# Cardinal-Cryptography/zk-apps

Measured on AMD Instinct MI355X. Metric: shielder_withdraw_groth16_proofs_per_sec_2^20_constraints, higher is better.
Workload: dtype int: signed 28-bit limbs in 32-bit words, 64-bit column accumulators (Fr 255-bit / Fq 381-bit Montgomery); 1 GPU; single withdraw-shaped Groth16 proof, N=2^20 (7 Fr NTTs, 4 G1 MSM + 1 G2 MSM of 2^20-1 terms), 1 proof per step per GPU; relation=update_note (withdraw) with Poseidon-5 hashing, chain-padded to N, curve=BLS12-381, independent_proofs_per_rank=173, distinct_witnesses_per_rank=64, fresh_r_s_per_proof=True, proofs_in_flight_per_gpu=3, msm_schedule=A | B1 (over r*z) + L + H reduced together | B2 (G2)

## Files before the change

zk-apps_amd/csrc/ntt.hip:

```cpp
#include <stdlib.h>
#include <type_traits>
#include <utility>
#include "ntt.hpp"
#include "tune.hpp"

namespace zkmi {

namespace {

__device__ __forceinline__ void ld_words8(const uint32_t* p, uint32_t* w) {
  const uint4* q = reinterpret_cast<const uint4*>(p);
  const uint4 a = q[0], b = q[1];
  w[0] = a.x; w[1] = a.y; w[2] = a.z; w[3] = a.w;
  w[4] = b.x; w[5] = b.y; w[6] = b.z; w[7] = b.w;
}
__device__ __forceinline__ void st_words8(uint32_t* p, const uint32_t* w) {
  uint4* q = reinterpret_cast<uint4*>(p);
  q[0] = make_uint4(w[0], w[1], w[2], w[3]);
  q[1] = make_uint4(w[4], w[5], w[6], w[7]);
}

template <class F>
__global__ void k_bitrev_copy(const F* __restrict__ in, F* __restrict__ out, int log_n) {
  const uint32_t i = blockIdx.x * blockDim.x + threadIdx.x;
  if (i >= (1u << log_n)) return;
  const uint32_t r = log_n ? (__brev(i) >> (32 - log_n)) : 0u;
  st28(out + r, ld28(in + i));
}

template <class F, bool DIF, bool LOCAL_TW, int THREADS>
__global__ void __launch_bounds__(THREADS)
k_ntt_pass(F* __restrict__ data, const F* __restrict__ tw, int log_n, int t0, int S, int Q,
           const F* __restrict__ post, uint32_t* __restrict__ canon_out) {
  data += (size_t)blockIdx.y << log_n;
  if (canon_out) canon_out += ((size_t)blockIdx.y << log_n) * 8;
  extern __shared__ __align__(16) unsigned char lds_raw[];
  F* tile = reinterpret_cast<F*>(lds_raw);
  const uint32_t tile_n = 1u << (S + Q);
  F* ctw = tile + tile_n;
  const uint32_t blk = blockIdx.x;
  const uint32_t mid_bits = (t0 > 0) ? (uint32_t)(t0 - Q) : 0u;
  const uint32_t mid = blk & ((1u << mid_bits) - 1u);
  const uint32_t hi = blk >> mid_bits;
  const uint32_t qeff = (t0 > 0) ? (uint32_t)Q : 0u;
  auto gindex = [&](uint32_t L) -> uint32_t {
    if (t0 == 0) return blk * tile_n + L;
    const uint32_t e = L >> Q, c = L & ((1u << Q) - 1u);
    return (hi << (t0 + S)) | (e << t0) | (mid << Q) | c;
  };
  auto twist = [&](uint32_t L) -> F {
    const uint32_t e = L >> Q, c = L & ((1u << Q) - 1u);
    const uint32_t col = (mid << Q) | c;
    const uint32_t ex = (col * (__brev(e) >> (32 - S))) << (log_n - t0 - S);
    const uint32_t halfn = 1u << (log_n - 1);
    F f = ld28(tw + (ex & (halfn - 1u)));
    return (ex & halfn) ? f.neg() : f;
  };
  if (LOCAL_TW)
    for (uint32_t k = threadIdx.x; k < (1u << (S - 1)); k += THREADS) ctw[k] = ld28(tw + ((size_t)k << (log_n - S)));
  for (uint32_t L = threadIdx.x; L < tile_n; L += THREADS) {
    F v = ld28(data + gindex(L));
    if (LOCAL_TW && !DIF && t0 > 0) v = v * twist(L);
    tile[L] = v;
  }
  __syncthreads();

  const uint32_t half = tile_n >> 1;
  for (int s = 0; s < S; s++) {
    const int u = DIF ? (S - 1 - s) : s;
    const int t = t0 + u;
    const uint32_t dist_log = (uint32_t)u + qeff;
    const uint32_t dist = 1u << dist_log;
    for (uint32_t b = threadIdx.x; b < half; b += THREADS) {
      const uint32_t lo = b & (dist - 1u);
      const uint32_t L0 = ((b >> dist_log) << (dist_log + 1)) | lo;
      const uint32_t L1 = L0 | dist;
      F w;
      if (LOCAL_TW) {
        w = ctw[(lo >> qeff) << (S - 1 - u)];
      } else {
        const uint32_t j = gindex(L0) & ((1u << t) - 1u);
        w = ld28(tw + ((size_t)j << (log_n - 1 - t)));
      }
      const F x = tile[L0];
      if (DIF) {
        const F y = tile[L1];
        tile[L0] = x + y;
        tile[L1] = x.sub_lazy(y) * w;
      } else {
        const F y = tile[L1] * w;
        tile[L0] = x + y;
        tile[L1] = x - y;
      }
    }
    __syncthreads();
  }

  for (uint32_t L = threadIdx.x; L < tile_n; L += THREADS) {
    const uint32_t g = gindex(L);
    F v = tile[L];
    if (LOCAL_TW && DIF && t0 > 0) v = v * twist(L);
    if (post) v = v * ld28(post + g);
    if (canon_out) {
      uint32_t w[8];
      v.to_canonical(w);
      st_words8(canon_out + (size_t)g * 8, w);
    } else {
      st28(data + g, v);
    }
  }
}

#ifdef ZKMI_EXPERIMENTS
#include "ntt_exp.hpp"
#endif

template <class F>
__global__ void __launch_bounds__(256)
k_mul_table(F* __restrict__ a, const F* __restrict__ b, uint32_t n) {
  const uint32_t i = blockIdx.x * blockDim.x + threadIdx.x;
  if (i < n) st28(a + i, ld28(a + i) * ld28(b + i));
}

template <class F>
__global__ void __launch_bounds__(256)
k_scale(F* __restrict__ a, F s, uint32_t n) {
  const uint32_t i = blockIdx.x * blockDim.x + threadIdx.x;
  if (i < n) st28(a + i, ld28(a + i) * s);
}

template <class F>
__global__ void __launch_bounds__(256)
k_power_table(F* __restrict__ out, F base, F first, uint32_t n) {
  const uint32_t i0 = (blockIdx.x * blockDim.x + threadIdx.x) * 16u;
  if (i0 >= n) return;
  F v = first, sq = base;
  for (uint32_t e = i0; e; e >>= 1) {
    if (e & 1u) v = v * sq;
    sq = sq * sq;
  }
  for (uint32_t k = 0; k < 16u && i0 + k < n; k++) {
    st28(out + i0 + k, v);
    v = v * base;
  }
}

template <class F>
__global__ void __launch_bounds__(256)
k_from_canonical(const uint32_t* __restrict__ in, F* __restrict__ out, uint32_t n) {
  const uint32_t i = blockIdx.x * blockDim.x + threadIdx.x;
  if (i >= n) return;
  uint32_t w[8];
  ld_words8(in + (size_t)i * 8, w);
  st28(out + i, F::from_canonical(w));
}
template <class F>
__global__ void __launch_bounds__(256)
k_to_canonical(const F* __restrict__ in, uint32_t* __restrict__ out, uint32_t n) {
  const uint32_t i = blockIdx.x * blockDim.x + threadIdx.x;
  if (i >= n) return;
  uint32_t w[8];
  ld28(in + i).to_canonical(w);
  st_words8(out + (size_t)i * 8, w);
}

}

Fr fr_root_of_unity(int log_n) {
  static const uint32_t ROOT_2_32[8] = {0x439f0d2bu, 0x3829971fu, 0x8c2280b9u, 0xb6368350u,
                                        0x22c813b4u, 0xd09b6819u, 0xdfe81f20u, 0x16a2a19eu};
  Fr w;
  for (int i = 0; i < 8; i++) w.l[i] = ROOT_2_32[i];
  w = w.to_mont();
  for (int i = 32; i > log_n; i--) w = w.sqr();
  return w;
}

NttField<Fr28>::Host NttField<Fr28>::root_max() { return fr_root_of_unity(32); }
NttField<BnFr28>::Host NttField<BnFr28>::root_max() {
  static const uint32_t ROOT_2_28[8] = {0x60c37c9cu, 0xd34f1ed9u, 0xd39329c8u, 0x3215cf6du,
                                        0x3dd31f74u, 0x98865ea9u, 0x166d18b7u, 0x03ddb9f5u};
  BnFr w;
  for (int i = 0; i < 8; i++) w.l[i] = ROOT_2_28[i];
  return w.to_mont();
}

template <class H>
static H host_from_u64(uint64_t v) {
  H a = H::zero();
  a.l[0] = (uint32_t)v;
  a.l[1] = (uint32_t)(v >> 32);
  return a.to_mont();
}
template <class F, class H>
static F to28(const H& a) {
  H c = a.from_mont();
  return F::from_canonical(c.l);
}

template <class F>
NttDomainT<F>::~NttDomainT() {
  F* ptrs[] = {tw_fwd, tw_inv, coset_fwd, coset_inv_n, rev_coset_n, rev_coset_inv_n, n_inv, scratch};
  for (F* p : ptrs)
    if (p) (void)hipFree(p);
}

template <class F>
hipError_t NttDomainT<F>::init(int log_n_, hipStream_t stream) {
  using H = typename NttField<F>::Host;
  if (log_n_ > NttField<F>::TWO_ADICITY) return hipErrorInvalidValue;
  log_n = log_n_;
  const uint32_t n = 1u << log_n;
  const uint32_t half = n > 1 ? n / 2 : 1;
  hipError_t e;
  F** alloc_n[] = {&coset_fwd, &coset_inv_n, &rev_coset_n, &rev_coset_inv_n, &scratch};
  if ((e = hipMalloc(&tw_fwd, sizeof(F) * half)) != hipSuccess) return e;
  if ((e = hipMalloc(&tw_inv, sizeof(F) * half)) != hipSuccess) return e;
  if ((e = hipMalloc(&n_inv, sizeof(F))) != hipSuccess) return e;
  for (F** p : alloc_n)
    if ((e = hipMalloc(p, sizeof(F) * n)) != hipSuccess) return e;
  H w = NttField<F>::root_max();
  for (int i = NttField<F>::TWO_ADICITY; i > log_n; i--) w = w.sqr();
  const H g = host_from_u64<H>(7);
  const H ninv = host_from_u64<H>(n).inv();
  const F one28 = F::one(), ninv28 = to28<F, H>(ninv);
  n_inv_host = ninv28;
  const int T = 256;
  auto blocks = [&](uint32_t cnt) { return (cnt + 16 * T - 1) / (16 * T); };
  hipLaunchKernelGGL(k_power_table<F>, dim3(blocks(half)), dim3(T), 0, stream, tw_fwd, to28<F, H>(w), one28, half);
  hipLaunchKernelGGL(k_power_table<F>, dim3(blocks(half)), dim3(T), 0, stream, tw_inv, to28<F, H>(w.inv()), one28, half);
  hipLaunchKernelGGL(k_power_table<F>, dim3(blocks(n)), dim3(T), 0, stream, coset_fwd, to28<F, H>(g), one28, n);
  hipLaunchKernelGGL(k_power_table<F>, dim3(blocks(n)), dim3(T), 0, stream, coset_inv_n, to28<F, H>(g.inv()), ninv28, n);
  hipLaunchKernelGGL(k_power_table<F>, dim3(blocks(n)), dim3(T), 0, stream, scratch, to28<F, H>(g), ninv28, n);
  hipLaunchKernelGGL(k_bitrev_copy<F>, dim3((n + T - 1) / T), dim3(T), 0, stream, scratch, rev_coset_n, log_n);
  hipLaunchKernelGGL(k_bitrev_copy<F>, dim3((n + T - 1) / T), dim3(T), 0, stream, coset_inv_n, rev_coset_inv_n, log_n);
  if ((e = hipMemcpyAsync(n_inv, &ninv28, sizeof(F), hipMemcpyHostToDevice, stream)) != hipSuccess) return e;
  if ((e = hipStreamSynchronize(stream)) != hipSuccess) return e;
  return hipGetLastError();
}

static int ntt_rb_mode() { return ZK_TUNE("ZKMI_NTT_RB", 6); }

#ifdef ZKMI_EXPERIMENTS
template <class F, bool DIF, bool LTW, int LOGE, int LOGR = 0, bool ONEW = false>
static void launch_rb(dim3 grid, uint32_t tile_n, int S, hipStream_t stream, F* buf, const F* tw, int log_n, int t0, int Q,
                      const F* post, uint32_t* canon_out) {
  const size_t words = (size_t)F::NL * (tile_n + (tile_n >> 5)) +
                       (LTW ? (size_t)F::NL * ((1u << (S - 1)) + ((1u << (S - 1)) >> 5) + 1u) : 0u);
  hipLaunchKernelGGL((k_ntt_pass_rb<F, DIF, LTW, LOGE, LOGR, ONEW>), grid, dim3(tile_n >> (LOGE + LOGR)), words * sizeof(uint32_t), stream,
                     buf, tw, log_n, t0, S, Q, post, canon_out);
}
#endif

template <class F, bool DIF>
static hipError_t run_passes(F* buf, const F* tw, int log_n, const F* post, uint32_t* canon_out,
                             hipStream_t stream, uint32_t batch = 1) {
  const uint32_t n = 1u << log_n;
  int mode = ntt_rb_mode();
  if (mode == 5 && log_n < 9) mode = 3;
  const int rb = (mode == 1 || mode == 2 || mode == 4 || mode == 5) ? mode : 0;
  const int tile_log = mode == 5 ? 9 : mode == 4 ? 10 : 11;
  struct Pass {
    int t0, S, Q;
  } passes[4];
  int np = 0;
  const int max_s = mode == 5 ? 9 : 10;
  const int want_np = (log_n + max_s - 1) / max_s;
  for (int t0 = 0; t0 < log_n;) {
    int S = log_n - t0;
    if (S > max_s) S = max_s;
    if (mode == 5) {
      const int left = want_np - np;
      S = (log_n - t0 + left - 1) / left;
    }
    int Q;
    if (rb) {
      Q = tile_log - S;
      const int room = (t0 > 0) ? t0 : (log_n - S);
      if (Q > room) Q = room;
    } else {
      Q = (t0 > 0) ? 1 : ((log_n > S) ? 1 : 0);
      if ((mode == 3 || mode == 6) && t0 > 0 && S < 10 && log_n - 11 >= 9) Q = (11 - S < t0) ? 11 - S : t0;
      if (mode == 6 && S + Q == 11) Q -= 1;
    }
    passes[np++] = {t0, S, Q};
    t0 += S;
  }
  const bool local3 = ZK_TUNE("ZKMI_NTT_LOCAL3", 0) == 1;
  const bool local_tw = np <= 2 || mode == 5 || local3;
  for (int k = 0; k < np; k++) {
    const Pass& p = DIF ? passes[np - 1 - k] : passes[k];
    const bool last = (k == np - 1);
    const uint32_t tile_n = 1u << (p.S + p.Q);
    const uint32_t nblk = n / tile_n;
    const F* pp = last ? post : nullptr;
    uint32_t* co = last ? canon_out : nullptr;
    const dim3 grid(nblk, batch);
#ifdef ZKMI_EXPERIMENTS
    if (rb == 5) {
      launch_rb<F, DIF, true, 2, 1, true>(grid, tile_n, p.S, stream, buf, tw, log_n, p.t0, p.Q, pp, co);
      continue;
    }
    if (rb == 4 && tile_n == 1024) {
      if (local_tw) launch_rb<F, DIF, true, 2, 2>(grid, tile_n, p.S, stream, buf, tw, log_n, p.t0, p.Q, pp, co);
      else launch_rb<F, DIF, false, 2, 2>(grid, tile_n, p.S, stream, buf, tw, log_n, p.t0, p.Q, pp, co);
      continue;
    }
    if (rb && rb != 4 && rb != 5 && tile_n >= 512) {
      if (rb == 2) {
        if (local_tw) launch_rb<F, DIF, true, 2>(grid, tile_n, p.S, stream, buf, tw, log_n, p.t0, p.Q, pp, co);
        else launch_rb<F, DIF, false, 2>(grid, tile_n, p.S, stream, buf, tw, log_n, p.t0, p.Q, pp, co);
      } else {
        if (local_tw) launch_rb<F, DIF, true, 3>(grid, tile_n, p.S, stream, buf, tw, log_n, p.t0, p.Q, pp, co);
        else launch_rb<F, DIF, false, 3>(grid, tile_n, p.S, stream, buf, tw, log_n, p.t0, p.Q, pp, co);
      }
      continue;
    }
#endif
    const size_t lds = ((size_t)tile_n + (local_tw ? (1u << (p.S - 1)) : 0u)) * sizeof(F);
    if (tile_n == 1024 && mode == 6) {
      if (local_tw)
        hipLaunchKernelGGL((k_ntt_pass<F, DIF, true, 512>), grid, dim3(512), lds, stream, buf, tw, log_n, p.t0, p.S, p.Q, pp, co);
      else
        hipLaunchKernelGGL((k_ntt_pass<F, DIF, false, 512>), grid, dim3(512), lds, stream, buf, tw, log_n, p.t0, p.S, p.Q, pp, co);
    } else if (tile_n >= 1024) {
      if (local_tw)
        hipLaunchKernelGGL((k_ntt_pass<F, DIF, true, 1024>), grid, dim3(1024), lds, stream, buf, tw, log_n, p.t0, p.S,
                           p.Q, pp, co);
      else
        hipLaunchKernelGGL((k_ntt_pass<F, DIF, false, 1024>), grid, dim3(1024), lds, stream, buf, tw, log_n, p.t0,
                           p.S, p.Q, pp, co);
    } else if (local_tw) {
      hipLaunchKernelGGL((k_ntt_pass<F, DIF, true, 64>), grid, dim3(64), lds, stream, buf, tw, log_n, p.t0, p.S, p.Q,
                         pp, co);
    } else {
      hipLaunchKernelGGL((k_ntt_pass<F, DIF, false, 64>), grid, dim3(64), lds, stream, buf, tw, log_n, p.t0, p.S, p.Q,
                         pp, co);
    }
  }
  return hipGetLastError();
}

template <class F>
hipError_t NttDomainT<F>::inverse_to_rev(F* d, const F* post_table, uint32_t* canon_out, hipStream_t st, uint32_t batch) {
  if (log_n == 0) {
    if (batch != 1) return hipErrorInvalidValue;
    if (post_table) hipLaunchKernelGGL(k_mul_table<F>, dim3(1), dim3(256), 0, st, d, post_table, 1u);
    if (canon_out) hipLaunchKernelGGL(k_to_canonical<F>, dim3(1), dim3(256), 0, st, d, canon_out, 1u);
    return hipGetLastError();
  }
  return run_passes<F, true>(d, tw_inv, log_n, post_table, canon_out, st, batch);
}

template <class F>
hipError_t NttDomainT<F>::forward_from_rev(F* d, hipStream_t st, uint32_t batch) {
  if (log_n == 0) return hipSuccess;
  return run_passes<F, false>(d, tw_fwd, log_n, nullptr, nullptr, st, batch);
}

template <class F>
hipError_t NttDomainT<F>::transform(F* d_data, bool inverse, bool coset, hipStream_t stream) {
  const uint32_t n = 1u << log_n;
  const int T = 256;
  if (coset && !inverse)
    hipLaunchKernelGGL(k_mul_table<F>, dim3((n + T - 1) / T), dim3(T), 0, stream, d_data, coset_fwd, n);
  if (log_n > 0) {
    hipLaunchKernelGGL(k_bitrev_copy<F>, dim3((n + T - 1) / T), dim3(T), 0, stream, d_data, scratch, log_n);
    hipError_t e = run_passes<F, false>(scratch, inverse ? tw_inv : tw_fwd, log_n, nullptr, nullptr, stream);
    if (e != hipSuccess) return e;
    if ((e = hipMemcpyAsync(d_data, scratch, sizeof(F) * n, hipMemcpyDeviceToDevice, stream)) != hipSuccess) return e;
  }
  if (inverse) {
    if (coset) {
      hipLaunchKernelGGL(k_mul_table<F>, dim3((n + T - 1) / T), dim3(T), 0, stream, d_data, coset_inv_n, n);
    } else {
      hipLaunchKernelGGL(k_scale<F>, dim3((n + T - 1) / T), dim3(T), 0, stream, d_data, n_inv_host, n);
    }
  }
  return hipGetLastError();
}

template <class F>
hipError_t ntt_from_canonical(const uint32_t* d_in, F* d_out, uint32_t n, hipStream_t s) {
  if (!n) return hipSuccess;
  hipLaunchKernelGGL(k_from_canonical<F>, dim3((n + 63) / 64), dim3(64), 0, s, d_in, d_out, n);
  return hipGetLastError();
}
template <class F>
hipError_t ntt_to_canonical(const F* d_in, uint32_t* d_out, uint32_t n, hipStream_t s) {
  if (!n) return hipSuccess;
  hipLaunchKernelGGL(k_to_canonical<F>, dim3((n + 255) / 256), dim3(256), 0, s, d_in, d_out, n);
  return hipGetLastError();
}
template <class F>
hipError_t ntt_mul_table(F* d, const F* table, uint32_t n, hipStream_t s) {
  if (!n) return hipSuccess;
  hipLaunchKernelGGL(k_mul_table<F>, dim3((n + 255) / 256), dim3(256), 0, s, d, table, n);
  return hipGetLastError();
}

#ifdef ZKMI_EXPERIMENTS
template <class F>
static hipError_t rb_enable_big_lds() {
  const void* fns[] = {reinterpret_cast<const void*>(k_ntt_pass_rb<F, true, true, 3>),  reinterpret_cast<const void*>(k_ntt_pass_rb<F, false, true, 3>),
                       reinterpret_cast<const void*>(k_ntt_pass_rb<F, true, false, 3>), reinterpret_cast<const void*>(k_ntt_pass_rb<F, false, false, 3>),
                       reinterpret_cast<const void*>(k_ntt_pass_rb<F, true, true, 2>),  reinterpret_cast<const void*>(k_ntt_pass_rb<F, false, true, 2>),
                       reinterpret_cast<const void*>(k_ntt_pass_rb<F, true, false, 2>), reinterpret_cast<const void*>(k_ntt_pass_rb<F, false, false, 2>),
                       reinterpret_cast<const void*>((k_ntt_pass_rb<F, true, true, 2, 2>)),  reinterpret_cast<const void*>((k_ntt_pass_rb<F, false, true, 2, 2>)),
                       reinterpret_cast<const void*>((k_ntt_pass_rb<F, true, false, 2, 2>)), reinterpret_cast<const void*>((k_ntt_pass_rb<F, false, false, 2, 2>)),
                       reinterpret_cast<const void*>((k_ntt_pass_rb<F, true, true, 2, 1, true>)), reinterpret_cast<const void*>((k_ntt_pass_rb<F, false, true, 2, 1, true>))};
  for (const void* f : fns) {
    const hipError_t e = hipFuncSetAttribute(f, hipFuncAttributeMaxDynamicSharedMemorySize, 160 * 1024);
    if (e != hipSuccess) return e;
  }
  return hipSuccess;
}
#endif

hipError_t ntt_enable_big_lds() {
  const void* fns[] = {reinterpret_cast<const void*>(k_ntt_pass<Fr28, true, true, 1024>),
                       reinterpret_cast<const void*>(k_ntt_pass<Fr28, false, true, 1024>),
                       reinterpret_cast<const void*>(k_ntt_pass<Fr28, true, false, 1024>),
                       reinterpret_cast<const void*>(k_ntt_pass<Fr28, false, false, 1024>),
                       reinterpret_cast<const void*>(k_ntt_pass<BnFr28, true, true, 1024>),
                       reinterpret_cast<const void*>(k_ntt_pass<BnFr28, false, true, 1024>),
                       reinterpret_cast<const void*>(k_ntt_pass<BnFr28, true, false, 1024>),
                       reinterpret_cast<const void*>(k_ntt_pass<BnFr28, false, false, 1024>),
                       reinterpret_cast<const void*>(k_ntt_pass<Fr28, true, true, 512>),
                       reinterpret_cast<const void*>(k_ntt_pass<Fr28, false, true, 512>),
                       reinterpret_cast<const void*>(k_ntt_pass<Fr28, true, false, 512>),
                       reinterpret_cast<const void*>(k_ntt_pass<Fr28, false, false, 512>),
                       reinterpret_cast<const void*>(k_ntt_pass<BnFr28, true, true, 512>),
                       reinterpret_cast<const void*>(k_ntt_pass<BnFr28, false, true, 512>),
                       reinterpret_cast<const void*>(k_ntt_pass<BnFr28, true, false, 512>),
                       reinterpret_cast<const void*>(k_ntt_pass<BnFr28, false, false, 512>)};
  for (const void* f : fns) {
    hipError_t e = hipFuncSetAttribute(f, hipFuncAttributeMaxDynamicSharedMemorySize, 160 * 1024);
    if (e != hipSuccess) return e;
  }
#ifdef ZKMI_EXPERIMENTS
  hipError_t e = rb_enable_big_lds<Fr28>();
  if (e == hipSuccess) e = rb_enable_big_lds<BnFr28>();
  return e;
#else
  return hipSuccess;
#endif
}

template struct NttDomainT<Fr28>;
template struct NttDomainT<BnFr28>;
template hipError_t ntt_from_canonical<Fr28>(const uint32_t*, Fr28*, uint32_t, hipStream_t);
template hipError_t ntt_to_canonical<Fr28>(const Fr28*, uint32_t*, uint32_t, hipStream_t);
template hipError_t ntt_mul_table<Fr28>(Fr28*, const Fr28*, uint32_t, hipStream_t);
template hipError_t ntt_from_canonical<BnFr28>(const uint32_t*, BnFr28*, uint32_t, hipStream_t);
template hipError_t ntt_to_canonical<BnFr28>(const BnFr28*, uint32_t*, uint32_t, hipStream_t);
template hipError_t ntt_mul_table<BnFr28>(BnFr28*, const BnFr28*, uint32_t, hipStream_t);

}
```

Baseline: 59.57 proofs/s.

## Use lazy limb reduction in NTT butterflies and fuse unit stages into load/store

NTT butterflies now use lazy add/sub on signed limbs and only carry-normalize every few stages (every 2 for DIF, every 3 for DIT), so most per-stage carry work is skipped. The twiddle-free unit-distance stage is folded into the global load (DIT) or the final store (DIF), which removes one LDS round-trip and one barrier per pass. Sign flips on twiddles become branchless XOR negation. This relies on the limb headroom being large enough for several unnormalized additions, and the multiply must accept unnormalized inputs.

```diff
diff --git a/zk-apps_amd/csrc/ntt.hip b/zk-apps_amd/csrc/ntt.hip
--- a/zk-apps_amd/csrc/ntt.hip
+++ b/zk-apps_amd/csrc/ntt.hip
@@ -26,6 +26,18 @@
   if (i >= (1u << log_n)) return;
   const uint32_t r = log_n ? (__brev(i) >> (32 - log_n)) : 0u;
   st28(out + r, ld28(in + i));
+}
+
+constexpr int NTT_DIF_SWEEP = 2;
+constexpr int NTT_DIT_SWEEP = 3;
+
+template <class F>
+__device__ __forceinline__ F neg_if_lazy(const F& f, bool sign) {
+  const int32_t m = sign ? -1 : 0;
+  F r;
+#pragma unroll
+  for (int i = 0; i < F::NL; i++) r.l[i] = (f.l[i] ^ m) - m;
+  return r;
 }
 
 template <class F, bool DIF, bool LOCAL_TW, int THREADS>
@@ -53,31 +65,49 @@
     const uint32_t col = (mid << Q) | c;
     const uint32_t ex = (col * (__brev(e) >> (32 - S))) << (log_n - t0 - S);
     const uint32_t halfn = 1u << (log_n - 1);
-    F f = ld28(tw + (ex & (halfn - 1u)));
-    return (ex & halfn) ? f.neg() : f;
+    return neg_if_lazy(ld28(tw + (ex & (halfn - 1u))), (ex & halfn) != 0u);
   };
+  const bool twisted = LOCAL_TW && t0 > 0;
+  const bool unit_stage = LOCAL_TW || t0 == 0;
+  const uint32_t half = tile_n >> 1;
+  const uint32_t unit_dist = 1u << qeff;
+  auto lower = [](uint32_t b, uint32_t dl) -> uint32_t { return ((b >> dl) << (dl + 1)) | (b & ((1u << dl) - 1u)); };
+  auto sweeps = [&](int s) -> bool { return (s + 1) % (DIF ? NTT_DIF_SWEEP : NTT_DIT_SWEEP) == 0 || s == S - 1; };
+
   if (LOCAL_TW)
     for (uint32_t k = threadIdx.x; k < (1u << (S - 1)); k += THREADS) ctw[k] = ld28(tw + ((size_t)k << (log_n - S)));
-  for (uint32_t L = threadIdx.x; L < tile_n; L += THREADS) {
-    F v = ld28(data + gindex(L));
-    if (LOCAL_TW && !DIF && t0 > 0) v = v * twist(L);
-    tile[L] = v;
+  if (!DIF && unit_stage) {
+    for (uint32_t b = threadIdx.x; b < half; b += THREADS) {
+      const uint32_t L0 = lower(b, qeff), L1 = L0 | unit_dist;
+      F x = ld28(data + gindex(L0)), y = ld28(data + gindex(L1));
+      if (twisted) {
+        x = x * twist(L0);
+        y = y * twist(L1);
+      }
+      F a = x.add_lazy(y), d = x.sub_lazy(y);
+      if (sweeps(0)) {
+        a.carry();
+        d.carry();
+      }
+      tile[L0] = a;
+      tile[L1] = d;
+    }
+  } else {
+    for (uint32_t L = threadIdx.x; L < tile_n; L += THREADS) tile[L] = ld28(data + gindex(L));
   }
   __syncthreads();
 
-  const uint32_t half = tile_n >> 1;
-  for (int s = 0; s < S; s++) {
+  auto stage = [&](int s, auto SWEEP) {
     const int u = DIF ? (S - 1 - s) : s;
     const int t = t0 + u;
     const uint32_t dist_log = (uint32_t)u + qeff;
     const uint32_t dist = 1u << dist_log;
     for (uint32_t b = threadIdx.x; b < half; b += THREADS) {
-      const uint32_t lo = b & (dist - 1u);
-      const uint32_t L0 = ((b >> dist_log) << (dist_log + 1)) | lo;
+      const uint32_t L0 = lower(b, dist_log);
       const uint32_t L1 = L0 | dist;
       F w;
       if (LOCAL_TW) {
-        w = ctw[(lo >> qeff) << (S - 1 - u)];
+        w = ctw[((L0 & (dist - 1u)) >> qeff) << (S - 1 - u)];
       } else {
         const uint32_t j = gindex(L0) & ((1u << t) - 1u);
         w = ld28(tw + ((size_t)j << (log_n - 1 - t)));
@@ -85,28 +115,65 @@
       const F x = tile[L0];
       if (DIF) {
         const F y = tile[L1];
-        tile[L0] = x + y;
+        F a = x.add_lazy(y);
+        if (decltype(SWEEP)::value) a.carry();
+        tile[L0] = a;
         tile[L1] = x.sub_lazy(y) * w;
       } else {
         const F y = tile[L1] * w;
-        tile[L0] = x + y;
-        tile[L1] = x - y;
+        F a = x.add_lazy(y), d = x.sub_lazy(y);
+        if (decltype(SWEEP)::value) {
+          a.carry();
+          d.carry();
+        }
+        tile[L0] = a;
+        tile[L1] = d;
       }
     }
     __syncthreads();
-  }
-
-  for (uint32_t L = threadIdx.x; L < tile_n; L += THREADS) {
-    const uint32_t g = gindex(L);
-    F v = tile[L];
-    if (LOCAL_TW && DIF && t0 > 0) v = v * twist(L);
-    if (post) v = v * ld28(post + g);
+  };
+  const int s_begin = (!DIF && unit_stage) ? 1 : 0, s_end = (DIF && unit_stage) ? S - 1 : S;
+  for (int s = s_begin; s < s_end; s++) {
+    if (sweeps(s)) stage(s, std::true_type());
+    else stage(s, std::false_type());
+  }
+
+  auto store = [&](uint32_t g, const F& v) {
     if (canon_out) {
       uint32_t w[8];
       v.to_canonical(w);
       st_words8(canon_out + (size_t)g * 8, w);
     } else {
       st28(data + g, v);
+    }
+  };
+  if (DIF && unit_stage) {
+    for (uint32_t b = threadIdx.x; b < half; b += THREADS) {
+      const uint32_t L0 = lower(b, qeff), L1 = L0 | unit_dist;
+      const uint32_t g0 = gindex(L0), g1 = gindex(L1);
+      const F x = tile[L0], y = tile[L1];
+      F a = x.add_lazy(y), d = x.sub_lazy(y);
+      if (twisted) {
+        a = a * twist(L0);
+        d = d * twist(L1);
+      }
+      if (post) {
+        a = a * ld28(post + g0);
+        d = d * ld28(post + g1);
+      }
+      if (!twisted && !post) {
+        a.carry();
+        d.carry();
+      }
+      store(g0, a);
+      store(g1, d);
+    }
+  } else {
+    for (uint32_t L = threadIdx.x; L < tile_n; L += THREADS) {
+      const uint32_t g = gindex(L);
+      F v = tile[L];
+      if (post) v = v * ld28(post + g);
+      store(g, v);
     }
   }
 }
```

Measured after the change: 59.05 proofs/s, median of 2. About the same (-0.9%).
